# baumgach/PHiSeg-code

Measured on AMD Instinct MI355X. Metric: training images/sec (ELBO step) phiseg_7_5 128x128 LIDC, higher is better.
Workload: dtype bf16; 1 GPU; phiseg_7_5 LIDC 128x128x1, 2 classes, bf16, batch norm, batch 64 per GPU, full ELBO training step (fwd + CE + KL + bwd + Adam); global_batch=64, parallelism=dp1

## Files before the change

include/phx.h:

```cpp
#ifndef PHX_H
#define PHX_H
#include <stddef.h>
#include <stdint.h>

#ifdef __cplusplus
extern "C" {
#endif

enum { PHX_F32 = 0, PHX_BF16 = 1 };
enum { PHX_ACT_ID = 0, PHX_ACT_RELU = 1, PHX_ACT_SOFTPLUS = 2 };
enum { PHX_OK = 0, PHX_E_INVAL = -1, PHX_E_SHAPE = -2, PHX_E_ALIGN = -3, PHX_E_LAUNCH = -4, PHX_E_RUNTIME = -5, PHX_E_COMM = -6 };

int phx_abi_version(void);
int phx_last_error(char* buf, size_t n);
int phx_crc32c(const void* data, size_t n, unsigned* crc);
int phx_device_info(int* cu_count, int* clock_khz, size_t* hbm_bytes, char* name, size_t name_n);
int phx_stream_create(void** stream);
int phx_stream_destroy(void* stream);
int phx_stream_sync(void* stream);
int phx_event_create(void** ev);
int phx_event_destroy(void* ev);
int phx_event_record(void* ev, void* stream);
int phx_event_sync(void* ev);
int phx_event_elapsed_ms(void* start, void* stop, float* ms);
// ... 217 lines not shown
int phx_upconv_supported(int B, int h, int w, int Cin, int Cout);
int phx_upconv_pack(const float* w_hwio, void* weff_fwd, void* weff_dgrad , void* wt_fwd, void* wt_dgrad ,
                    const float* bias, float* bias4, int Cin, int Cout, void* stream);
int phx_upconv_fold_wgrad(const float* dweff, const float* dwt , float* dw_hwio, int Cin, int Cout, void* stream);
int phx_upconv_frame_gather(const void* x, void* f_rows, void* f_cols, int B, int h, int w, int C, void* stream);
int phx_upconv_frame_scatter(const void* fr, const void* fc, void* y_packed, int B, int h, int w, int Cout, void* stream);
int phx_upconv_frame_gather_dy(void* dy_packed, void* dfr, void* dfc, int B, int h, int w, int Cout, void* stream);
int phx_upconv_frame_scatter_dx(const void* df_rows, const void* df_cols, void* dx, int B, int h, int w, int C, void* stream);
int phx_norm_apply_fused_d2s(const void* x, int x_dt, const float* sums, const float* pivot, const float* gamma, const float* beta, float eps,
                             void* y, int y_dt, float* mean, float* rstd, float* scale, float* shift, float* moving_mean, float* moving_var,
                             float momentum, int NS, int P, int C, int G, int act, int h, int w, void* stream);
int phx_norm_bwd_reduce_s2d(const void* dA, int da_dt, const void* x, int x_dt, const float* scale, const float* shift,
                            const float* mean, const float* rstd, float* sums2, int NS, int P, int C, int G, int act, int nrep, int h,
                            int w, void* stream);
int phx_norm_bwd_apply_fused_s2d(const void* dA, int da_dt, const void* x, int x_dt, const float* scale, const float* shift,
                                 const float* mean, const float* rstd, const float* gamma, const float* sums2, void* dx, int dx_dt,
                                 float* dgamma, float* dbeta, const float* fwd_sums, const float* fwd_pivot, float* dbias, int NS, int P,
                                 int C, int G, int act, int nrep, int h, int w, void* stream);
int phx_depth_to_space2(const void* packed, void* hi, int B, int h, int w, int C, void* stream);
int phx_space_to_depth2(const void* hi, void* packed, int B, int h, int w, int C, void* stream);
int phx_bilinear_up2x_fwd(const void* x, int dt, void* y, int B, int h, int w, int C, void* stream);
int phx_bilinear_up2x_bwd(const void* dy, int dt, void* dx, int B, int h, int w, int C, void* stream);
int phx_bilinear_up2x_bwd_acc(const void* dy, int dt, void* dx, int B, int h, int w, int C, void* stream);
int phx_concat2(const void* a, int Ca, const void* b, int Cb, void* out, size_t npix, int dt, void* stream);
int phx_split2(const void* in, void* a, int Ca, void* b, int Cb, size_t npix, int dt, void* stream);
int phx_add_inplace(void* dst, const void* src, size_t n, int dt, void* stream);
int phx_channel_sum_accumulate(const void* x, int dt, float* out, size_t npix, int C, void* stream);
int phx_cast(const void* src, int src_dt, void* dst, int dst_dt, size_t n, void* stream);
int phx_posterior_input(const float* x, const uint8_t* s, void* out, int out_dt, size_t npix, int nlabels,
                        void* stream);
int phx_global_avgpool_fwd(const float* x, float* y, int B, int P, int C, void* stream);
int phx_global_avgpool_bwd(const float* dy, float* dx, int B, int P, int C, void* stream);
int phx_broadcast_pixels_fwd(const float* z, void* out, int out_dt, int B, int P, int C, void* stream);
int phx_broadcast_pixels_bwd(const void* dout, int dt, float* dz, int B, int P, int C, void* stream);
int phx_recomb_samples(const void* feat, int feat_dt, const float* z, const float* W0, const float* W1, const float* W2,
                       const float* W3, const float* b3, const float* s0, const float* t0, const float* s1, const float* t1,
                       const float* s2, const float* t2, float* logits, float* sm, int B, int n, int P, int KF, int K, int Z, int C,
                       void* stream);

int phx_reparam_fwd(const float* mu, const float* sigma, float* z, int B, int per_sample, uint64_t seed,
                    const int32_t* step_dev, int stream_id, int sample_offset, void* stream);
int phx_reparam_bwd(const float* dz, float* dsigma, int B, int per_sample, uint64_t seed,
                    const int32_t* step_dev, int stream_id, int sample_offset, void* stream);
int phx_philox_normal(float* out, int B, int per_sample, uint64_t seed, const int32_t* step_dev, int stream_id,
                      int sample_offset, void* stream);

// ... 112 lines not shown
```

phiseg_code_amd/engine.py:

```python
import ctypes
import os

import numpy as np
import torch

from phiseg_code_amd import graph as G
from phiseg_code_amd import optimizers
from phiseg_code_amd import runtime as rt
from phiseg_code_amd.tfwrapper import normalisation as tfnorm

from phiseg_code_amd.engine_common import *
from phiseg_code_amd.engine_common import (_BN_SMALL, _BN_SMALL_F32, _DETERMINISTIC, _NREP, _NREP_MINP, _fgn_mode, _dual_enabled, _noop,
                                           _device, _TORCH_DT, _NP_DT, _ESIZE, _LIK_SIDE_MAXLVL, _WGRAD_DEFER_BLOCKS, _STAMPS)
from phiseg_code_amd.engine_backward import BackwardLowering
from phiseg_code_amd.engine_forward import ForwardLowering


class ParamStore:

    def __init__(self, graph, seed=0, live=None, optimizer=None):
        self.graph = graph
        self.offset, self.state_offset = {}, {}
        off = soff = 0
        names = list(graph.variables)
# ... 439 lines not shown
        if with_bw:
            self._emit(self.L.memset, self.store.grads.data_ptr(), 0, self.store.grads.numel() * 4, self.stream)
        if self._stamp_tagged:
            for k in range(16):
                self._cur.append((self.L.stamp, (self._tstamp_buf.data_ptr() + 8 * k, self.stream)))
        nl = len(self._lanes)
        self.op_lane = {op: self._lane_of(op) for op in ops}
        opset = set(ops)
        self._opset = opset
        self._lat = self._find_latent_heads(ops)
        self._kl_group = None
        kls = [op for op in ops if op.type == "kl"]
        if len(kls) >= 2 and len(kls) <= 8:
            ws = [self.loss_weight.get(op.outputs[0], 0.0) for op in kls]
            i0, i1 = ops.index(kls[0]), ops.index(kls[-1])
            between = [op for op in ops[i0:i1 + 1] if op.type != "kl"]
            if (len({self.op_lane[op] for op in kls}) == 1 and all(abs(w - ws[0]) < 1e-12 for w in ws)
                    and not any(i.op in kls for b in between for i in b.inputs)):
                self._kl_group = dict(ops=kls, recs=[], gscale=ws[0])
        self._bw_skip = set()
        self._norm_head = {}
        self._pool_done = set()
        self._recomb = self._find_recomb_chains(ops)
        fork = self._record(0) if nl > 1 else None
        for ln in range(1, nl):
            self._lane = ln
            self._wait(fork)
        if nl > 1:
            self._touch = torch.zeros(64, dtype=torch.int64, device=_device())
            self._keep.append(self._touch)
            toks = []
            for ln in range(1, nl):
                self._lane = ln
                self._emit(self.L.stamp, self._touch.data_ptr() + 8 * ln, self.stream)
                toks.append(self._record(ln))
            self._lane = 0
            for evl in toks:
                self._wait(evl)
        self.fw_event = {}
        for op in ops:
            ln = self._lane = self.op_lane[op]
            for t in op.inputs:
                self._wait(self.fw_event.get(self._real_producer(t)))
            n0 = len(self._cur)
            self._stamp_begin()
            if op in self._recomb:
# ... 203 lines not shown
```

phiseg_code_amd/engine_backward.py:

```python
import ctypes

import numpy as np

from phiseg_code_amd import runtime as rt
from phiseg_code_amd import upconv
from phiseg_code_amd.engine_common import *
from phiseg_code_amd.engine_common import _HEAD_RIDER_NOUT, _BN_SMALL, _BN_SMALL_F32, _BN_WIDE, _BN_WIDE_MAXLINES, _DETERMINISTIC, _NREP, _NREP_MINP, _fgn_mode, _dual_enabled, _noop, _device, _TORCH_DT, _NP_DT, _ESIZE, _LIK_SIDE_MAXLVL, _WGRAD_DEFER_BLOCKS, _STAMPS


class BackwardLowering:
    def _bw_l2_weights(self, op):
        st = self.store
        self._emit(self.L.axpy_masked, st.grads.data_ptr(), st.params.data_ptr(), st.decay_mask.data_ptr(), st.n_train,
                   float(self._l2_weight), self.stream)

    def _bw_latent_group(self, rec):
        mu_op, sig_op, add_op = rec["mu"], rec["sig"], rec["add"]
        mu_t, sig_t = mu_op.outputs[0], sig_op.outputs[0]
        for t in (mu_t, sig_t):
            if t in self.grad:
                self._finalize_grad(t)
        dz = self.grad.get(add_op.outputs[0]) if add_op is not None else None
        dmu, dsg = self.grad.get(mu_t), self.grad.get(sig_t)
        for o in (mu_op, sig_op, add_op):
            if o is not None:
                self._bw_skip.add(o)
        if dz is None and dmu is None and dsg is None:
            return
        x_t = rec["x"]
        x, sigma = self.val[x_t], self.val[sig_t]
        npix, cin, zd = rec["npix"], rec["cin"], rec["zd"]
        gmu, gsig = self._alloc((npix, zd), F32), self._alloc((npix, zd), F32)
        st, Lb = self.store, self.L
        wmu, wsg = mu_op.attrs["W"], sig_op.attrs["W"]
        if not self.req.get(x_t, False):
            raise NotImplementedError("latent heads on a tensor without gradient")

        def wr(g):
            self._emit(Lb.latent_heads_bwd, dz.ptr if dz is not None else None, dmu.ptr if dmu is not None else None,
                       dsg.ptr if dsg is not None else None, sigma.ptr, st.ptr(wmu), st.ptr(wsg), g.ptr, g.dt, gmu.ptr, gsig.ptr, npix,
                       cin, zd, rec["hw"], self.rng_seed, self._noise_step_ptr(), rec["sid"], self.sample_offset, self.stream)
        self._add_grad(x_t, write_fn=wr)
        for hop, gy in ((mu_op, gmu), (sig_op, gsig)):
            W, b = hop.attrs["W"], hop.attrs["b"]
# ... 47 lines not shown
            op = op.inputs[0].op
        return op

    def _real_consumers(self, t, opset):
        out = []
        for c in t.consumers:
            if c not in opset:
                continue
            if c.type in self._VIRTUAL:
                for o in c.outputs:
                    out.extend(self._real_consumers(o, opset))
            else:
                out.append(c)
        return out

    def _finalize_grad(self, t):
        for buf, evl in self.pending.pop(t, []):
            self._wait(evl)
            g = self.grad[t]
            if buf is not g:
                assert g.dt == buf.dt and g.n == buf.n
                self._emit(self.L.add_inplace, g.ptr, buf.ptr, g.n, g.dt, self.stream)

    def _bw_placeholder(self, op):
        pass


    _bw_one_hot = _bw_sub_const = _bw_random_normal = _bw_mul = _bw_weighted_sum = _bw_constant = _bw_dice_table = _bw_placeholder

    def _resize_adjoint(self, dfine, dst, add):
        B, h, w, C = dst.shape
        assert dfine.dt == F32 and dst.dt == F32 and dfine.shape[1] % h == 0
        self._emit(self.L.nn_resize_adjoint, dfine.ptr, dst.ptr, B, h, w, C, (dfine.shape[1] // h).bit_length() - 1, int(add), self.stream)

    def _bw_nn_resize(self, op):
        d, src = self.grad[op.outputs[0]], self.val[op.inputs[0]]
        if op.attrs["shift"] == 0:
            return self._add_grad(op.inputs[0], buf=d)
        assert d.shape[1] == src.shape[1] << op.attrs["shift"], "the gradient of a resized tensor is taken at full resolution"
        self._add_grad(op.inputs[0], write_fn=lambda g: self._resize_adjoint(d, g, False), accum_fn=lambda g: self._resize_adjoint(d, g, True))

    def _bw_residual_ce(self, op):
        sv = self.saved.get(op)
        if sv:
            g = self.grad.get(op.outputs[op.attrs["L"]])
            if g is not None:
# ... 23 lines not shown
        sv = self.saved.get(op)
        if sv:
            lg, lab = self.val[op.inputs[0]], self.val[op.inputs[1]]
            B, H, W, C = lg.shape

            def emit(g, add):
                self._emit(self.L.dice_grad, lg.ptr, lab.ptr, sv["coef"].ptr, sv["gscale"], add, g.ptr, B, H, W, C, self.stream)
            self._add_grad(op.inputs[0], write_fn=lambda g: emit(g, 0), accum_fn=lambda g: emit(g, 1))

    def _bw_seg_xent(self, op):
        sv = self.saved.get(op)
        if sv:
            self._add_grad(op.inputs[0], buf=sv["d"])

    def _bw_kl(self, op):
        sv = self.saved.get(op)
        if sv:
            for t, g in zip(op.inputs, sv["gs"]):
                self._add_grad(t, buf=g)

    def _bw_add(self, op):
        if op in self._lat:
            return self._bw_latent_group(self._lat[op])
        sv, dz = self.saved[op], self.grad[op.outputs[0]]
        self._add_grad(sv["mu_t"], buf=dz)
        B = dz.shape[0]

        def wr(target):
            self._emit(self.L.reparam_bwd, dz.ptr, target.ptr, B, sv["per"], self.rng_seed,
                       self._noise_step_ptr(), sv["stream_id"], self.sample_offset, self.stream)
        self._add_grad(sv["sigma_t"], write_fn=wr)

    def _bw_concat(self, op):
        a, b = op.inputs
        d = self.grad[op.outputs[0]]
        if b.op.type == "sub_const":
            return
        npix = int(np.prod(d.shape[:-1]))
        ca, cb = self.val[a].shape[-1], self.val[b].shape[-1]
        da = self._alloc(self.val[a].shape, d.dt) if self.req.get(a) else None
        db = self._alloc(self.val[b].shape, d.dt) if self.req.get(b) else None
        self._emit(self.L.split2, d.ptr, da.ptr if da else None, ca, db.ptr if db else None, cb, npix, d.dt,
                   self.stream)
        for t, g in ((a, da), (b, db)):
            if g is not None:
                self._add_grad(t, buf=self._as_dt(g, self.val[t].dt))
# ... 350 lines not shown
            wsb = int(Lb.conv3x3_mfma_ws_bytes(B, H, Wd, cout, cin))
            ws = self._alloc((wsb // 4,), F32) if wsb else None
            self._emit(Lb.conv3x3_mfma_bf16_ws, dY.ptr, wd.ptr, g.ptr if g is not None else None, None, 0, None, ws.ptr if ws else None, wsb,
                       B, H, Wd, cout, cin, S, **dtag)
            return ws
        if isinstance(x, DualBuf):
            ta, tb = xin.op.inputs
            _, wd = self._packed(W)
            g1, g2 = self._alloc(x.a.shape, BF16), self._alloc(x.b.shape, BF16)
            wsb = int(Lb.conv3x3_mfma_ws_bytes(B, H, Wd, cout, cin))
            ws = self._alloc((wsb // 4,), F32) if wsb else None
            self._emit(Lb.conv3x3_mfma_bf16_dual, dY.ptr, None, 0, wd.ptr, g1.ptr, g2.ptr, x.k1, None, None, 0, None, 0,
                       ws.ptr if ws else None, wsb, B, H, Wd, cout, cin, S, **dtag)
            for t, gb in ((ta, g1), (tb, g2)):
                if self.req.get(t, False):
                    self._add_grad(t, buf=gb)
        elif sv.norm_head:
            self._add_grad(xin, buf=HeadGrad(self.val[xin], dY, self.store.ptr(W), cout))
        elif sv.head1x1:
            self._add_grad(xin, write_fn=lambda g: self._emit(
                Lb.head1x1_dgrad, dY.ptr, self.store.ptr(W), g.ptr, g.dt, B * H * Wd, cin, cout, S))
        elif sv.padded:
            ce, wdp = sv.cin_eff, sv.wd_pad

            def wr(g):
                inplace = ce == cin and g.dt == BF16
                gp = g if inplace else self._alloc((B, H, Wd, ce), BF16)
                self._emit(Lb.conv3x3_mfma_bf16, dY.ptr, wdp.ptr, gp.ptr, None, 0, None, B, H, Wd, cout, ce, S, **dtag)
                if not inplace:
                    self._emit(Lb.unpad_channels_bf16, gp.ptr, g.ptr, g.dt, cin, ce, B * H * Wd, S)
            self._add_grad(xin, write_fn=wr)
        elif sv.mfma and self._slice_grad_ok(op, xin, B, H, Wd, cout, cin):
            _, wd = self._packed(W)
            ws = mfma_dgrad(None)
            self._add_grad(xin, buf=SliceGrad(self.val[xin], ws, int(Lb.conv3x3_mfma_ksplit(B, H, Wd, cout, cin))))
        elif sv.mfma:
            _, wd = self._packed(W)
            self._add_grad(xin, write_fn=mfma_dgrad)
        elif sv.f32m and cin % 32 == 0 and dY.dt == F32 and self._wpk32.get(W.name, (None, None))[1] is not None:
            wd32 = self._wpk32[W.name][1]

            def wr_f32m(g):
                assert g.dt == F32
                self._emit(Lb.conv3x3_f32_mfma, dY.ptr, wd32.ptr, None, g.ptr, B, H, Wd, cout, cin, 0, S,
                           tag="conv3x3_f32_mfma_dgrad", flops=18.0 * cin * cout * B * H * Wd)
            self._add_grad(xin, write_fn=wr_f32m)
# ... 5 lines not shown
```

phiseg_code_amd/engine_common.py:

```python
import ctypes
import enum
import os

import numpy as np
import torch

from phiseg_code_amd import graph as G
from phiseg_code_amd import runtime as rt
from phiseg_code_amd.tfwrapper import normalisation as tfnorm

__all__ = ['F32', 'BF16', 'U8', '_TORCH_DT', '_NP_DT', '_ESIZE', '_LIK_SIDE_MAXLVL', '_WGRAD_DEFER_BLOCKS', '_NREP', '_NREP_MINP', '_STAMPS', '_DETERMINISTIC', '_BN_SMALL', '_BN_SMALL_F32', '_BN_WIDE', '_BN_WIDE_MAXLINES', '_SKIP_HEAD_A', '_POOL_FUSE', '_xf_enabled', '_upconv_min_h', 'UpBuf', '_fgn_mode', '_dual_enabled', '_f32_mfma_enabled', '_recomb_enabled', '_onepass_enabled', '_head_rider_enabled', '_HEAD_RIDER_NOUT', '_noop', '_device', 'live_variables', 'device_sync', 'Buf', 'DualBuf', 'HeadGrad', 'SliceGrad', 'XfBuf', 'NormRoute', 'StatsSource', 'ConvSaved', 'RenormSaved']

F32, BF16, U8 = rt.F32, rt.BF16, 2
_TORCH_DT = {F32: torch.float32, BF16: torch.bfloat16, U8: torch.uint8}
_NP_DT = {F32: np.float32, U8: np.uint8}
_ESIZE = {F32: 4, BF16: 2, U8: 1}
_LIK_SIDE_MAXLVL = 3
_WGRAD_DEFER_BLOCKS = 96
_NREP = 4
_NREP_MINP = 4096
_STAMPS = os.environ.get("PHX_STAMPS", "0") == "1"
_DETERMINISTIC = os.environ.get("PHX_DETERMINISTIC", "0") not in ("0", "")
_BN_SMALL = 1024
_BN_SMALL_F32 = True
_BN_WIDE_MAXLINES = 2048
_SKIP_HEAD_A = True
_POOL_FUSE = True
_BN_WIDE = 2


def _fgn_mode():
    return int(os.environ.get("PHX_FGN", "1"))


def _upconv_min_h():
    return int(os.environ.get("PHX_UPCONV", "64"))


def _xf_enabled():
    return os.environ.get("PHX_XF", "1") == "1"


def _dual_enabled():
    return os.environ.get("PHX_DUAL", "1") == "1"


def _recomb_enabled():
    return os.environ.get("PHX_RECOMB", "1") == "1"


def _f32_mfma_enabled():
    return os.environ.get("PHX_F32_MFMA", "1") == "1"


def _onepass_enabled():
    return os.environ.get("PHX_ONEPASS", "1") == "1"


_HEAD_RIDER_NOUT = (2, 4)


def _head_rider_enabled():
    return os.environ.get("PHX_HEAD_RIDER", "1") != "0"


def _noop():
    pass
# ... 77 lines not shown
    def __init__(self, like, ws, nz):
        self.shape, self.dt, self.n = like.shape, like.dt, like.n
        self.ws, self.nz = ws, nz


class XfBuf:

    def __init__(self, like, y, scale, shift):
        self.shape, self.dt, self.n = like.shape, like.dt, like.n
        self.y, self.scale, self.shift = y, scale, shift


class UpBuf:

    def __init__(self, src, shape):
        self.src, self.shape, self.dt = src, tuple(int(v) for v in shape), src.dt
        self.n = int(np.prod(self.shape))

    @property
    def nbytes(self):
        return self.n * _ESIZE[self.dt]


class RenormSaved:
    __slots__ = ("r", "d", "gamma_eff", "dgs", "dbs")

    def __init__(self, r, d, gamma_eff, dgs=None, dbs=None):
        self.r, self.d, self.gamma_eff, self.dgs, self.dbs = r, d, gamma_eff, dgs, dbs


class NormRoute(enum.Enum):
    NONE, INFER_FOLDED, INFER, BN_WIDE, BN_SMALL_F32Y, BN_SMALL, FGN, NORM_SMALL, GENERIC, RENORM_SMALL = range(10)


class StatsSource(enum.Enum):
    PARTIALS, PARTIALS_NS, ATOMIC, DIRECT, PIVOT_PASS = range(5)


class ConvSaved:
    _OPTIONAL = dict(route=NormRoute.NONE, y=None, scale=None, shift=None, mean=None, rstd=None, NS=None, P=None, G=None, wd_pad=None,
                     upconv=None, a_unwritten=None, fsums=None, fpivot=None, transposed=None, general=None, geo=None, f32m=False,
                     norm_head=False, latent=False, renorm=None)
    __slots__ = ("x", "out", "norm", "mfma", "padded", "cin_eff", "k1", "head1x1") + tuple(_OPTIONAL)

    def __init__(self, x, out, norm, mfma, padded, cin_eff, k1, head1x1, **optional):
        self.x, self.out, self.norm, self.mfma, self.padded, self.cin_eff, self.k1, self.head1x1 = x, out, norm, mfma, padded, cin_eff, k1, head1x1
# ... 9 lines not shown
```

phiseg_code_amd/engine_forward.py:

```python
import ctypes
import types

import numpy as np
import torch

from phiseg_code_amd import graph as G
from phiseg_code_amd import runtime as rt
from phiseg_code_amd import upconv
from phiseg_code_amd.tfwrapper import normalisation as tfnorm
from phiseg_code_amd.engine_common import *
from phiseg_code_amd.engine_common import _BN_SMALL, _BN_SMALL_F32, _BN_WIDE, _BN_WIDE_MAXLINES, _SKIP_HEAD_A, _DETERMINISTIC, _NREP, _NREP_MINP, _fgn_mode, _dual_enabled, _recomb_enabled, _noop, _device, _TORCH_DT, _NP_DT, _ESIZE, _LIK_SIDE_MAXLVL, _WGRAD_DEFER_BLOCKS, _STAMPS


def conv_norm_route(Lb, norm, training, bw, act_dt, x_dt, y_dt, out_dt, B, H, Wd, cin_eff, cout, Gn, mfma, head1x1, concat_free, upsampled,
                    deterministic=_DETERMINISTIC, fgn=None):
    fgn = _fgn_mode() if fgn is None else fgn
    if norm is None:
        return NormRoute.NONE, None
    per_batch = norm in ("batch", "renorm")
    NS, P = (1, B * H * Wd) if per_batch else (B, H * Wd)
    if norm == "batch" and not training:
        return (NormRoute.INFER_FOLDED if (mfma and not head1x1 and not bw) else NormRoute.INFER), None
    both_bf16 = y_dt == BF16 and out_dt == BF16
    if norm == "renorm" and both_bf16 and P <= _BN_SMALL and Lb.renorm_small_supported(P, cout, y_dt, out_dt):
# ... 257 lines not shown
                     for t in (mu.outputs[0], sig.outputs[0]) for c in t.consumers if c in opset)
            ok = ok and len({self.op_lane[o] for o in members}) == 1
            if not ok:
                continue
            rec = dict(mu=mu, sig=sig, add=add, last=last, x=x)
            for o in members:
                out[o] = rec
        return out

    def _fw_latent_group(self, rec):
        mu_op, sig_op, add_op = rec["mu"], rec["sig"], rec["add"]
        x = self.val[rec["x"]]
        mu, sigma = self.val[mu_op.outputs[0]], self.val[sig_op.outputs[0]]
        z = self.val[add_op.outputs[0]] if add_op is not None else None
        cin, zd = mu_op.attrs["W"].shape[-2], mu_op.attrs["W"].shape[-1]
        npix = int(np.prod(x.shape[:-1]))
        hw = npix // x.shape[0]
        sid = add_op.inputs[1].op.inputs[1].op.attrs["stream"] if add_op is not None else 0
        st = self.store
        self._emit(self.L.latent_heads_fwd, x.ptr, x.dt, st.ptr(mu_op.attrs["W"]), st.ptr(mu_op.attrs["b"]), st.ptr(sig_op.attrs["W"]),
                   st.ptr(sig_op.attrs["b"]), mu.ptr, sigma.ptr, z.ptr if z is not None else None, npix, cin, zd, hw, self.rng_seed,
                   self._noise_step_ptr(), sid, self.sample_offset, self.stream)
        rec.update(npix=npix, hw=hw, sid=sid, cin=cin, zd=zd)

    def _find_recomb_chains(self, ops):
        out = {}
        if self.loss is not None or not _recomb_enabled():
            return out
        opset = set(ops)

        def sole_reader(t):
            cons = [c for c in t.consumers if c in opset]
            return cons[0] if (len(cons) == 1 and t not in self.fetches and t not in self.fed) else None

        def plain_1x1(op):
            a = op.attrs
            return (op.type == "conv_unit" and a.get("transposed") is None and a.get("general") is None and a["ksize"] == 1
                    and op not in self._lat)
        for tb in ops:
            if tb.type != "tile_batch" or len(tb.inputs[0].shape) != 4:
                continue
            KF = tb.inputs[0].shape[-1]
            if KF not in (32, 64):
                continue
            cat = sole_reader(tb.outputs[0])
            if cat is None or cat.type != "concat" or cat.inputs[0] is not tb.outputs[0] or cat.inputs[1].op.type != "tile_pixels":
# ... 141 lines not shown
            sv.y = o.y

    def _conv_operands(self, op, bw):
        a = op.attrs
        x = self.val[op.inputs[0]]
        W, b = a["W"], a["b"]
        k, (_, _, cin, cout) = a["ksize"], W.shape
        B, H, Wd = x.shape[0], x.shape[1], x.shape[2]
        out = self._alloc_like(op.outputs[0])
        self.val[op.outputs[0]] = out
        mfma = (self.act_dt == BF16 and x.dt == BF16 and out.dt == BF16 and k == 3 and cin % 32 == 0
                and cout % 32 == 0)
        dual = x if isinstance(x, DualBuf) else None
        assert dual is None or mfma, "concat-free input reached a convolution off the MFMA path"
        up = x if isinstance(x, UpBuf) else None
        xf = x if isinstance(x, XfBuf) else None
        assert xf is None or (mfma and a["norm"] == "batch" and b is None), "unmaterialised activation reached a convolution that cannot re-form it"
        cin_eff = cin
        k1 = k == 1 and cout % 32 == 0
        padded = (self.act_dt == BF16 and out.dt == BF16 and cout % 32 == 0 and
                  ((k == 3 and (cin % 32 != 0 or x.dt != BF16)) or k1))
        if padded:
            cin_eff = (cin + 31) // 32 * 32
            if cin_eff != cin or x.dt != BF16:
                xp = self._alloc((B, H, Wd, cin_eff), BF16)
                self._emit(self.L.pad_channels_bf16, x.ptr, x.dt, cin, xp.ptr, cin_eff, B * H * Wd, self.stream)
                x = xp
            mfma = True
        head1x1 = (k == 1 and out.dt == F32 and cout in (2, 4, 6, 8) and a["norm"] is None and b is not None)
        f32m = bool(not mfma and self.act_dt == F32 and x.dt == F32 and out.dt == F32 and k == 3 and cout % 32 == 0 and _f32_mfma_enabled()
                    and isinstance(x, Buf) and self.L.conv3x3_f32_mfma_supported(B, H, Wd, cin, cout))
        training = a["training"] if isinstance(a["training"], bool) else self.training
        sv = ConvSaved(x, out, self._lowered_norm(a, training), mfma, padded, cin_eff, bool(padded and k1), head1x1, f32m=f32m)
        wptr, wf = self.store.ptr(W), None
        if padded:
            wf = self._alloc((9 * cin_eff * cout,), BF16)
            sv.wd_pad = self._alloc((9 * cin_eff * cout,), BF16) if (bw and self.req.get(op.inputs[0], False)) else None
            self._pack_jobs.append((wptr, wf.ptr, sv.wd_pad.ptr if sv.wd_pad else 0, cin, cin_eff, cout, 1 if k1 else 0))
        elif mfma:
            wf, _ = self._packed(W)
        return types.SimpleNamespace(op=op, a=a, bw=bw, sv=sv, x=x, out=out, W=W, k=k, cin=cin, cout=cout, B=B, H=H, Wd=Wd, dual=dual, up=up, xf=xf,
                                     wf=wf, wptr=wptr, bptr=self.store.ptr(b) if b is not None else None, act=rt.ACT_CODES[a["act"]],
                                     training=training,
                                     y=None, sums=None, pivot=None, stats=None, apply_args=None)

    def _mfma_conv(self, o, y, bias_p, oscale_p, act_code, stats, stats_mode, ws, wsb):
        Lb, x, xf, dual = self.L, o.x, o.xf, o.dual
# ... 276 lines not shown
        mh = _upconv_min_h()
        if not (mh > 0 and bw and self.loss is not None and self.act_dt == BF16 and isinstance(x, Buf) and x.dt == BF16 and len(x.shape) == 4):
            return None
        ot = op.outputs[0]
        cons = self._real_consumers(ot, self._opset)
        if len(cons) != 1 or ot in self.fetches or x.shape[1] < max(mh, 32) or x.shape[2] < max(mh, 32):
            return None
        c = cons[0]
        a = c.attrs if c.type == "conv_unit" else None
        if (a is None or c.inputs[0] is not ot or a["ksize"] != 3 or a.get("transposed") is not None or a.get("general") is not None
                or a["norm"] not in ("batch", "group", "instance") or (a["norm"] == "batch") != (a["b"] is None)
                or self.op_lane.get(c) != self.op_lane.get(op) or c in self._lat):
            return None
        training = a["training"] if isinstance(a["training"], bool) else self.training
        cin, cout = a["W"].shape[-2], a["W"].shape[-1]
        if not training or cin != x.shape[3] or not self.L.upconv_supported(x.shape[0], x.shape[1], x.shape[2], cin, cout):
            return None
        if cin < 4 * cout:
            return None
        return c

    def _fw_bilinear_up(self, op, bw):
        x = self.val[op.inputs[0]]
        if self._upconv_consumer(op, x, bw) is not None:
            self.val[op.outputs[0]] = UpBuf(x, self._cshape(op.outputs[0]))
            return
        out = self._alloc(self._cshape(op.outputs[0]), x.dt)
        self.val[op.outputs[0]] = out
        self._emit(self.L.bilinear_up2x_fwd, x.ptr, x.dt, out.ptr, x.shape[0], x.shape[1], x.shape[2], x.shape[3],
                   self.stream)

    def _fw_add(self, op, bw):
        if op.outputs[0] in self.fed:
            t = op.outputs[0]
            z = self._alloc(self._cshape(t), F32, zero=True)
            self.val[t] = z
            self.feeds[t] = z
            return
        mu_t, m = op.inputs
        if m.op.type != "mul" or m.op.inputs[1].op.type != "random_normal":
            raise NotImplementedError("only z = mu + sigma * random_normal(...) is on the hot path")
        rec = self._lat.get(op)
        if rec is not None:
            self.val[op.outputs[0]] = self._alloc(self.val[mu_t].shape, F32)
            self.saved[op] = dict(latent=True)
            if rec["last"] is op:
                self._fw_latent_group(rec)
            return
        sigma_t, eps_t = m.op.inputs
        mu, sigma = self.val[mu_t], self.val[sigma_t]
        z = self._alloc(mu.shape, F32)
        self.val[op.outputs[0]] = z
        per = mu.n // mu.shape[0]
        stream_id = eps_t.op.attrs["stream"]
        self._emit(self.L.reparam_fwd, mu.ptr, sigma.ptr, z.ptr, mu.shape[0], per, self.rng_seed,
                   self._noise_step_ptr(), stream_id, self.sample_offset, self.stream)
        self.saved[op] = dict(mu_t=mu_t, sigma_t=sigma_t, per=per, stream_id=stream_id)

    def _fw_tile_batch(self, op, bw):
        x = self.val[op.inputs[0]]
        out = self._alloc(self._cshape(op.outputs[0]), x.dt)
        self.val[op.outputs[0]] = out
        n = op.attrs["tile"]
        assert out.shape[0] == x.shape[0] * n
        per = x.n // x.shape[0]
        if (per * _ESIZE[x.dt]) % 16 and x.dt == F32:
            self._emit(self.L.broadcast_pixels_fwd, x.ptr, out.ptr, F32, x.shape[0], n, per, self.stream)
            return
        self._emit(self.L.repeat_batch, x.ptr, out.ptr, x.shape[0], (x.n // x.shape[0]) * _ESIZE[x.dt], n, self.stream)

    def _fw_global_avgpool(self, op, bw):
        x = self._as_dt(self.val[op.inputs[0]], F32)
        out = self._alloc_like(op.outputs[0])
        self.val[op.outputs[0]] = out
        self._emit(self.L.global_avgpool_fwd, x.ptr, out.ptr, x.shape[0], x.shape[1] * x.shape[2], x.shape[3],
                   self.stream)

    def _fw_tile_pixels(self, op, bw):
        z = self.val[op.inputs[0]]
        out = self._alloc_like(op.outputs[0])
# ... 152 lines not shown
```

Before: 6625 images/s.

## Fuse latent z fan-out (pad + bilinear upsample) and gradient fan-in into glue kernels

Adds zglue kernels. In the forward pass, one kernel writes each sampled latent z both as a channel-padded bf16 map and as a 2x bilinear-upsampled padded map, replacing the separate pad_channels and bilinear_up launches that fed the 3x3 convolutions. In the backward pass, the data-gradient outputs of those convolutions are gathered into a single fan-in kernel that applies the upsample adjoint and sums all sources into dz, with cross-lane events. This cuts launches and intermediate buffers on the small latent paths, at the cost of extra engine bookkeeping and cross-lane waits.

```diff
diff --git a/include/phx.h b/include/phx.h
--- a/include/phx.h
+++ b/include/phx.h
@@ -263,6 +263,11 @@
 int phx_bilinear_up2x_fwd(const void* x, int dt, void* y, int B, int h, int w, int C, void* stream);
 int phx_bilinear_up2x_bwd(const void* dy, int dt, void* dx, int B, int h, int w, int C, void* stream);
 int phx_bilinear_up2x_bwd_acc(const void* dy, int dt, void* dx, int B, int h, int w, int C, void* stream);
+enum { PHX_Z_FANIN_MAX = 4 };
+enum { PHX_Z_SRC_DENSE = 0, PHX_Z_SRC_PAD = 1, PHX_Z_SRC_UP = 2 };
+int phx_z_fanout(const float* z, void* zpad, void* zup, int B, int h, int w, int Z, int Cpad, void* stream);
+int phx_z_fanin(const void* const* srcs, const int* kinds, const int* separate, int nsrc, float* dz, int B, int h, int w, int Z, int Cpad,
+                void* stream);
 int phx_concat2(const void* a, int Ca, const void* b, int Cb, void* out, size_t npix, int dt, void* stream);
 int phx_split2(const void* in, void* a, int Ca, void* b, int Cb, size_t npix, int dt, void* stream);
 int phx_add_inplace(void* dst, const void* src, size_t n, int dt, void* stream);
diff --git a/phiseg_code_amd/csrc/zglue.hip b/phiseg_code_amd/csrc/zglue.hip
--- /dev/null
+++ b/phiseg_code_amd/csrc/zglue.hip
@@ -0,0 +1,281 @@
+#include "phx_common.h"
+
+template <int Z>
+__device__ __forceinline__ void zg_load_f32(const float* __restrict__ p, float o[Z]) {
+    const float2* q = reinterpret_cast<const float2*>(p);
+#pragma unroll
+    for (int j = 0; j < Z / 2; ++j) {
+        const float2 t = q[j];
+        o[2 * j] = t.x;
+        o[2 * j + 1] = t.y;
+    }
+}
+template <int Z>
+__device__ __forceinline__ void zg_load_pad(const unsigned short* __restrict__ p, float o[Z]) {
+    const uint4 r = *reinterpret_cast<const uint4*>(p);
+    const unsigned w[4] = {r.x, r.y, r.z, r.w};
+#pragma unroll
+    for (int j = 0; j < Z / 2; ++j) {
+        o[2 * j] = __uint_as_float(w[j] << 16);
+        o[2 * j + 1] = __uint_as_float(w[j] & 0xffff0000u);
+    }
+}
+template <int Z>
+__device__ __forceinline__ uint4 zg_chunk0(const float v[Z]) {
+    unsigned w[4] = {0u, 0u, 0u, 0u};
+#pragma unroll
+    for (int j = 0; j < Z / 2; ++j) w[j] = (unsigned)f2bf(v[2 * j]) | ((unsigned)f2bf(v[2 * j + 1]) << 16);
+    return make_uint4(w[0], w[1], w[2], w[3]);
+}
+
+template <int Z>
+__global__ void k_z_fanout(const float* __restrict__ z, unsigned short* __restrict__ zpad, unsigned short* __restrict__ zup, int B, int h,
+                           int w, int Cpad) {
+    const int Q = Cpad / 8, OW = 2 * w;
+    const size_t items = (size_t)B * h * w * Q;
+    for (size_t it = blockIdx.x * (size_t)blockDim.x + threadIdx.x; it < items; it += (size_t)gridDim.x * blockDim.x) {
+        const int q = (int)(it % Q);
+        size_t r = it / Q;
+        const size_t pix = r;
+        const int x0 = (int)(r % w); r /= w;
+        const int y0 = (int)(r % h);
+        const size_t base = (r / h) * h;
+        uint4 c00 = make_uint4(0u, 0u, 0u, 0u), c01 = c00, c10 = c00, c11 = c00, cz = c00;
+        if (q == 0) {
+            float a[Z];
+            zg_load_f32<Z>(z + pix * Z, a);
+            cz = zg_chunk0<Z>(a);
+            if (zup) {
+                const int y1 = min(y0 + 1, h - 1), x1 = min(x0 + 1, w - 1);
+                float bb[Z], c[Z], d[Z], o00[Z], o01[Z], o10[Z], o11[Z];
+                zg_load_f32<Z>(z + ((base + y0) * w + x1) * Z, bb);
+                zg_load_f32<Z>(z + ((base + y1) * w + x0) * Z, c);
+                zg_load_f32<Z>(z + ((base + y1) * w + x1) * Z, d);
+#pragma unroll
+                for (int j = 0; j < Z; ++j) {
+                    const float top = fmaf(bb[j] - a[j], 0.5f, a[j]);
+                    const float bot = fmaf(d[j] - c[j], 0.5f, c[j]);
+                    o00[j] = fmaf(c[j] - a[j], 0.f, a[j]);
+                    o01[j] = fmaf(bot - top, 0.f, top);
+                    o10[j] = fmaf(c[j] - a[j], 0.5f, a[j]);
+                    o11[j] = fmaf(bot - top, 0.5f, top);
+                }
+                c00 = zg_chunk0<Z>(o00);
+                c01 = zg_chunk0<Z>(o01);
+                c10 = zg_chunk0<Z>(o10);
+                c11 = zg_chunk0<Z>(o11);
+            }
+        }
+        if (zpad) *reinterpret_cast<uint4*>(zpad + pix * Cpad + (size_t)q * 8) = cz;
+        if (zup) {
+            const size_t o = ((base * 2 + 2 * y0) * OW + 2 * x0) * Cpad + (size_t)q * 8;
+            *reinterpret_cast<uint4*>(zup + o) = c00;
+            *reinterpret_cast<uint4*>(zup + o + Cpad) = c01;
+            *reinterpret_cast<uint4*>(zup + o + (size_t)OW * Cpad) = c10;
+            *reinterpret_cast<uint4*>(zup + o + (size_t)OW * Cpad + Cpad) = c11;
+        }
+    }
+}
+
+struct ZFanInArgs {
+    const void* src[PHX_Z_FANIN_MAX];
+    int kind[PHX_Z_FANIN_MAX];
+    int separate[PHX_Z_FANIN_MAX];
+    int n;
+};
+
+template <int Z>
+__device__ __forceinline__ void zg_adjoint(const unsigned short* __restrict__ dy, int b, int iy, int ix, int h, int w, int Cpad, float acc[Z]) {
+    const int OH = 2 * h, OW = 2 * w;
+    int ty[3], tx[3];
+    float wy[3], wx[3];
+    ty[0] = 2 * iy; wy[0] = 1.f;
+    ty[1] = 2 * iy + 1; wy[1] = (iy == h - 1) ? 1.f : 0.5f;
+    ty[2] = 2 * iy - 1; wy[2] = (iy >= 1) ? 0.5f : 0.f;
+    tx[0] = 2 * ix; wx[0] = 1.f;
+    tx[1] = 2 * ix + 1; wx[1] = (ix == w - 1) ? 1.f : 0.5f;
+    tx[2] = 2 * ix - 1; wx[2] = (ix >= 1) ? 0.5f : 0.f;
+    for (int a = 0; a < 3; ++a) {
+        if (wy[a] == 0.f) continue;
+        for (int c = 0; c < 3; ++c) {
+            if (wx[c] == 0.f) continue;
+            float v[Z];
+            zg_load_pad<Z>(dy + (((size_t)b * OH + ty[a]) * OW + tx[c]) * Cpad, v);
+            const float ww = wy[a] * wx[c];
+#pragma unroll
+            for (int j = 0; j < Z; ++j) acc[j] = fmaf(ww, v[j], acc[j]);
+        }
+    }
+}
+
+template <int Z>
+__global__ void k_z_fanin(const ZFanInArgs A, float* __restrict__ dz, int B, int h, int w, int Cpad) {
+    const size_t items = (size_t)B * h * w;
+    for (size_t it = blockIdx.x * (size_t)blockDim.x + threadIdx.x; it < items; it += (size_t)gridDim.x * blockDim.x) {
+        size_t r = it;
+        const int ix = (int)(r % w); r /= w;
+        const int iy = (int)(r % h);
+        const int b = (int)(r / h);
+        float acc[Z];
+#pragma unroll
+        for (int j = 0; j < Z; ++j) acc[j] = 0.f;
+        for (int k = 0; k < A.n; ++k) {
+            if (A.kind[k] == PHX_Z_SRC_UP) {
+                const unsigned short* dy = (const unsigned short*)A.src[k];
+                if (k == 0 || !A.separate[k]) {
+                    zg_adjoint<Z>(dy, b, iy, ix, h, w, Cpad, acc);
+                } else {
+                    float t[Z];
+#pragma unroll
+                    for (int j = 0; j < Z; ++j) t[j] = 0.f;
+                    zg_adjoint<Z>(dy, b, iy, ix, h, w, Cpad, t);
+#pragma unroll
+                    for (int j = 0; j < Z; ++j) acc[j] = acc[j] + t[j];
+                }
+            } else {
+                float v[Z];
+                if (A.kind[k] == PHX_Z_SRC_DENSE) zg_load_f32<Z>((const float*)A.src[k] + it * Z, v);
+                else zg_load_pad<Z>((const unsigned short*)A.src[k] + it * Cpad, v);
+#pragma unroll
+                for (int j = 0; j < Z; ++j) acc[j] = k == 0 ? v[j] : acc[j] + v[j];
+            }
+        }
+        float2* o = reinterpret_cast<float2*>(dz + it * Z);
+#pragma unroll
+        for (int j = 0; j < Z / 2; ++j) o[j] = make_float2(acc[2 * j], acc[2 * j + 1]);
+    }
+}
+
+template <int Z, int NS>
+__global__ void __launch_bounds__(64) k_z_fanin_pk(const ZFanInArgs A, float* __restrict__ dz, int B, int h, int w, int Cpad) {
+    const size_t items = (size_t)B * h * w;
+    for (size_t it = blockIdx.x * (size_t)blockDim.x + threadIdx.x; it < items; it += (size_t)gridDim.x * blockDim.x) {
+        size_t r = it;
+        const int ix = (int)(r % w); r /= w;
+        const int iy = (int)(r % h);
+        const int b = (int)(r / h);
+        const int ty[3] = {2 * iy, 2 * iy + 1, max(2 * iy - 1, 0)}, tx[3] = {2 * ix, 2 * ix + 1, max(2 * ix - 1, 0)};
+        const float wy[3] = {1.f, (iy == h - 1) ? 1.f : 0.5f, (iy >= 1) ? 0.5f : 0.f};
+        const float wx[3] = {1.f, (ix == w - 1) ? 1.f : 0.5f, (ix >= 1) ? 0.5f : 0.f};
+        uint4 raw[NS][9];
+#pragma unroll
+        for (int k = 0; k < NS; ++k) {
+            const bool up = A.kind[k] == PHX_Z_SRC_UP;
+            const unsigned short* p = (const unsigned short*)A.src[k];
+            const int HH = up ? 2 * h : h, WW = up ? 2 * w : w;
+#pragma unroll
+            for (int a = 0; a < 3; ++a)
+#pragma unroll
+                for (int c = 0; c < 3; ++c) {
+                    const int yy = up ? ty[a] : iy, xx = up ? tx[c] : ix;
+                    raw[k][3 * a + c] = *reinterpret_cast<const uint4*>(p + (((size_t)b * HH + yy) * WW + xx) * Cpad);
+                }
+        }
+        float acc[Z];
+#pragma unroll
+        for (int j = 0; j < Z; ++j) acc[j] = 0.f;
+#pragma unroll
+        for (int k = 0; k < NS; ++k) {
+            const bool up = A.kind[k] == PHX_Z_SRC_UP, own = up && k > 0 && A.separate[k];
+            float t[Z];
+#pragma unroll
+            for (int j = 0; j < Z; ++j) t[j] = (up && !own) ? acc[j] : 0.f;
+            if (up) {
+#pragma unroll
+                for (int a = 0; a < 3; ++a)
+#pragma unroll
+                    for (int c = 0; c < 3; ++c) {
+                        const float ww = wy[a] * wx[c];
+                        const unsigned wd[4] = {raw[k][3 * a + c].x, raw[k][3 * a + c].y, raw[k][3 * a + c].z, raw[k][3 * a + c].w};
+                        if (wy[a] != 0.f && wx[c] != 0.f) {
+#pragma unroll
+                            for (int j = 0; j < Z / 2; ++j) {
+                                t[2 * j] = fmaf(ww, __uint_as_float(wd[j] << 16), t[2 * j]);
+                                t[2 * j + 1] = fmaf(ww, __uint_as_float(wd[j] & 0xffff0000u), t[2 * j + 1]);
+                            }
+                        }
+                    }
+            } else {
+                const unsigned wd[4] = {raw[k][0].x, raw[k][0].y, raw[k][0].z, raw[k][0].w};
+#pragma unroll
+                for (int j = 0; j < Z / 2; ++j) {
+                    t[2 * j] = __uint_as_float(wd[j] << 16);
+                    t[2 * j + 1] = __uint_as_float(wd[j] & 0xffff0000u);
+                }
+            }
+#pragma unroll
+            for (int j = 0; j < Z; ++j) acc[j] = (k == 0 || (up && !own)) ? t[j] : acc[j] + t[j];
+        }
+        float2* o = reinterpret_cast<float2*>(dz + it * Z);
+#pragma unroll
+        for (int j = 0; j < Z / 2; ++j) o[j] = make_float2(acc[2 * j], acc[2 * j + 1]);
+    }
+}
+
+#define PHX_Z_SWITCH(Z, ZC, ...)                  \
+    do {                                           \
+        if ((Z) == 2) { constexpr int ZC = 2; __VA_ARGS__; }      \
+        else if ((Z) == 4) { constexpr int ZC = 4; __VA_ARGS__; } \
+        else { constexpr int ZC = 6; __VA_ARGS__; }               \
+    } while (0)
+
+static int zglue_domain(int B, int h, int w, int Z, int Cpad) {
+    PHX_REQUIRE(B >= 1 && h >= 1 && w >= 1, PHX_E_INVAL, "z glue: empty map");
+    PHX_REQUIRE(Z == 2 || Z == 4 || Z == 6, PHX_E_INVAL, "z glue: Z must be 2, 4 or 6");
+    PHX_REQUIRE(Cpad == 32, PHX_E_INVAL, "z glue: Cpad must be 32");
+    return PHX_OK;
+}
+
+extern "C" {
+
+int phx_z_fanout(const float* z, void* zpad, void* zup, int B, int h, int w, int Z, int Cpad, void* stream) {
+    const int rc = zglue_domain(B, h, w, Z, Cpad);
+    if (rc != PHX_OK) return rc;
+    PHX_REQUIRE(z != NULL && (zpad != NULL || zup != NULL), PHX_E_INVAL, "z_fanout: z and at least one output");
+    PHX_REQUIRE(((uintptr_t)z & 7) == 0 && (((uintptr_t)zpad | (uintptr_t)zup) & 15) == 0, PHX_E_ALIGN, "z_fanout: z 8-byte, outputs 16-byte aligned");
+    const size_t items = (size_t)B * h * w * (Cpad / 8);
+    PHX_Z_SWITCH(Z, ZC, {
+        hipLaunchKernelGGL((k_z_fanout<ZC>), dim3(phx_grid_for(items, 256)), dim3(256), 0, (hipStream_t)stream, z, (unsigned short*)zpad,
+                           (unsigned short*)zup, B, h, w, Cpad);
+    });
+    PHX_CHECK_LAUNCH();
+    return PHX_OK;
+}
+
+int phx_z_fanin(const void* const* srcs, const int* kinds, const int* separate, int nsrc, float* dz, int B, int h, int w, int Z, int Cpad,
+                void* stream) {
+    const int rc = zglue_domain(B, h, w, Z, Cpad);
+    if (rc != PHX_OK) return rc;
+    PHX_REQUIRE(srcs != NULL && kinds != NULL && separate != NULL && dz != NULL && nsrc >= 1 && nsrc <= PHX_Z_FANIN_MAX, PHX_E_INVAL,
+                "z_fanin: 1 to PHX_Z_FANIN_MAX sources");
+    PHX_REQUIRE(((uintptr_t)dz & 7) == 0, PHX_E_ALIGN, "z_fanin: dz 8-byte aligned");
+    ZFanInArgs A;
+    memset(&A, 0, sizeof(A));
+    A.n = nsrc;
+    for (int k = 0; k < nsrc; ++k) {
+        PHX_REQUIRE(srcs[k] != NULL && kinds[k] >= PHX_Z_SRC_DENSE && kinds[k] <= PHX_Z_SRC_UP, PHX_E_INVAL, "z_fanin: bad source");
+        PHX_REQUIRE(((uintptr_t)srcs[k] & (kinds[k] == PHX_Z_SRC_DENSE ? 7 : 15)) == 0, PHX_E_ALIGN,
+                    "z_fanin: dense sources 8-byte, padded sources 16-byte aligned");
+        A.src[k] = srcs[k];
+        A.kind[k] = kinds[k];
+        A.separate[k] = separate[k] != 0;
+    }
+    const size_t items = (size_t)B * h * w;
+    bool dense = false;
+    for (int k = 0; k < nsrc; ++k) dense = dense || kinds[k] == PHX_Z_SRC_DENSE;
+    static_assert(PHX_Z_FANIN_MAX == 4, "the dispatch below lists the source counts");
+    const dim3 grid(phx_grid_for(items, 64)), block(64);
+#define PHX_Z_FANIN_PK(NSC) hipLaunchKernelGGL((k_z_fanin_pk<ZC, NSC>), grid, block, 0, (hipStream_t)stream, A, dz, B, h, w, Cpad)
+    PHX_Z_SWITCH(Z, ZC, {
+        if (dense) hipLaunchKernelGGL((k_z_fanin<ZC>), grid, block, 0, (hipStream_t)stream, A, dz, B, h, w, Cpad);
+        else if (nsrc == 1) PHX_Z_FANIN_PK(1);
+        else if (nsrc == 2) PHX_Z_FANIN_PK(2);
+        else if (nsrc == 3) PHX_Z_FANIN_PK(3);
+        else PHX_Z_FANIN_PK(4);
+    });
+#undef PHX_Z_FANIN_PK
+    PHX_CHECK_LAUNCH();
+    return PHX_OK;
+}
+
+}
diff --git a/phiseg_code_amd/engine.py b/phiseg_code_amd/engine.py
--- a/phiseg_code_amd/engine.py
+++ b/phiseg_code_amd/engine.py
@@ -485,6 +485,7 @@
         self._norm_head = {}
         self._pool_done = set()
         self._recomb = self._find_recomb_chains(ops)
+        self._zg, self._zg_conv, self._zg_up = self._find_zglue(ops)
         fork = self._record(0) if nl > 1 else None
         for ln in range(1, nl):
             self._lane = ln
diff --git a/phiseg_code_amd/engine_backward.py b/phiseg_code_amd/engine_backward.py
--- a/phiseg_code_amd/engine_backward.py
+++ b/phiseg_code_amd/engine_backward.py
@@ -20,6 +20,8 @@
         for t in (mu_t, sig_t):
             if t in self.grad:
                 self._finalize_grad(t)
+        if add_op is not None:
+            self._zglue_fanin(add_op.outputs[0])
         dz = self.grad.get(add_op.outputs[0]) if add_op is not None else None
         dmu, dsg = self.grad.get(mu_t), self.grad.get(sig_t)
         for o in (mu_op, sig_op, add_op):
@@ -113,6 +115,29 @@
                 assert g.dt == buf.dt and g.n == buf.n
                 self._emit(self.L.add_inplace, g.ptr, buf.ptr, g.n, g.dt, self.stream)
 
+    def _zglue_source(self, rec, gp, how):
+        t, srcs, lane = rec["t"], rec["sources"], self._lane
+        primary = not srcs or (how == "up" and all(s["lane"] == lane for s in srcs if s["primary"]))
+        evl = self._record(lane) if len(self._lanes) > 1 else None
+        srcs.append(dict(buf=gp, kind=2 if how == "up" else 1, primary=primary, lane=lane, evl=evl))
+        if t not in self.grad:
+            self.grad[t] = self._alloc(self.val[t].shape, F32)
+
+    def _zglue_fanin(self, t):
+        rec = self._zg.get(t)
+        if rec is None or not rec["sources"]:
+            return
+        srcs = [s for s in rec["sources"] if s["primary"]] + [s for s in rec["sources"] if not s["primary"]]
+        rec["sources"] = []
+        for s in srcs:
+            self._wait(s["evl"])
+        dz = self.grad[t]
+        B, h, w, Z = dz.shape
+        ptrs, kinds = rt.ptr_array([s["buf"].ptr for s in srcs]), rt.int_array([s["kind"] for s in srcs])
+        sep = rt.int_array([0 if s["primary"] else 1 for s in srcs])
+        self._keep += [ptrs, kinds, sep]
+        self._emit(self.L.z_fanin, ptrs, kinds, sep, len(srcs), dz.ptr, B, h, w, Z, 32, self.stream)
+
     def _bw_placeholder(self, op):
         pass
 
@@ -182,6 +207,7 @@
     def _bw_add(self, op):
         if op in self._lat:
             return self._bw_latent_group(self._lat[op])
+        self._zglue_fanin(op.outputs[0])
         sv, dz = self.saved[op], self.grad[op.outputs[0]]
         self._add_grad(sv["mu_t"], buf=dz)
         B = dz.shape[0]
@@ -578,6 +604,11 @@
                 Lb.head1x1_dgrad, dY.ptr, self.store.ptr(W), g.ptr, g.dt, B * H * Wd, cin, cout, S))
         elif sv.padded:
             ce, wdp = sv.cin_eff, sv.wd_pad
+            zg = self._zg_conv.get(op)
+            if zg is not None and zg[0]["bw"]:
+                gp = self._alloc((B, H, Wd, ce), BF16)
+                self._emit(Lb.conv3x3_mfma_bf16, dY.ptr, wdp.ptr, gp.ptr, None, 0, None, B, H, Wd, cout, ce, S, **dtag)
+                return self._zglue_source(zg[0], gp, zg[1])
 
             def wr(g):
                 inplace = ce == cin and g.dt == BF16
diff --git a/phiseg_code_amd/engine_common.py b/phiseg_code_amd/engine_common.py
--- a/phiseg_code_amd/engine_common.py
+++ b/phiseg_code_amd/engine_common.py
@@ -9,7 +9,7 @@
 from phiseg_code_amd import runtime as rt
 from phiseg_code_amd.tfwrapper import normalisation as tfnorm
 
-__all__ = ['F32', 'BF16', 'U8', '_TORCH_DT', '_NP_DT', '_ESIZE', '_LIK_SIDE_MAXLVL', '_WGRAD_DEFER_BLOCKS', '_NREP', '_NREP_MINP', '_STAMPS', '_DETERMINISTIC', '_BN_SMALL', '_BN_SMALL_F32', '_BN_WIDE', '_BN_WIDE_MAXLINES', '_SKIP_HEAD_A', '_POOL_FUSE', '_xf_enabled', '_upconv_min_h', 'UpBuf', '_fgn_mode', '_dual_enabled', '_f32_mfma_enabled', '_recomb_enabled', '_onepass_enabled', '_head_rider_enabled', '_HEAD_RIDER_NOUT', '_noop', '_device', 'live_variables', 'device_sync', 'Buf', 'DualBuf', 'HeadGrad', 'SliceGrad', 'XfBuf', 'NormRoute', 'StatsSource', 'ConvSaved', 'RenormSaved']
+__all__ = ['F32', 'BF16', 'U8', '_TORCH_DT', '_NP_DT', '_ESIZE', '_LIK_SIDE_MAXLVL', '_WGRAD_DEFER_BLOCKS', '_NREP', '_NREP_MINP', '_STAMPS', '_DETERMINISTIC', '_BN_SMALL', '_BN_SMALL_F32', '_BN_WIDE', '_BN_WIDE_MAXLINES', '_SKIP_HEAD_A', '_POOL_FUSE', '_xf_enabled', '_upconv_min_h', 'UpBuf', '_fgn_mode', '_dual_enabled', '_f32_mfma_enabled', '_recomb_enabled', '_zglue_enabled', 'ZUpBuf', '_onepass_enabled', '_head_rider_enabled', '_HEAD_RIDER_NOUT', '_noop', '_device', 'live_variables', 'device_sync', 'Buf', 'DualBuf', 'HeadGrad', 'SliceGrad', 'XfBuf', 'NormRoute', 'StatsSource', 'ConvSaved', 'RenormSaved']
 
 F32, BF16, U8 = rt.F32, rt.BF16, 2
 _TORCH_DT = {F32: torch.float32, BF16: torch.bfloat16, U8: torch.uint8}
@@ -43,6 +43,10 @@
 
 def _dual_enabled():
     return os.environ.get("PHX_DUAL", "1") == "1"
+
+
+def _zglue_enabled():
+    return os.environ.get("PHX_ZGLUE", "1") == "1"
 
 
 def _recomb_enabled():
@@ -166,6 +170,13 @@
         return self.n * _ESIZE[self.dt]
 
 
+class ZUpBuf:
+
+    def __init__(self, pad, shape):
+        self.pad, self.shape, self.dt = pad, tuple(int(v) for v in shape), F32
+        self.n = int(np.prod(self.shape))
+
+
 class RenormSaved:
     __slots__ = ("r", "d", "gamma_eff", "dgs", "dbs")
 
diff --git a/phiseg_code_amd/engine_forward.py b/phiseg_code_amd/engine_forward.py
--- a/phiseg_code_amd/engine_forward.py
+++ b/phiseg_code_amd/engine_forward.py
@@ -303,6 +303,61 @@
                    st.ptr(sig_op.attrs["b"]), mu.ptr, sigma.ptr, z.ptr if z is not None else None, npix, cin, zd, hw, self.rng_seed,
                    self._noise_step_ptr(), sid, self.sample_offset, self.stream)
         rec.update(npix=npix, hw=hw, sid=sid, cin=cin, zd=zd)
+        if add_op is not None:
+            self._zglue_fanout(add_op.outputs[0])
+
+    def _find_zglue(self, ops):
+        zg, by_conv, by_up = {}, {}, {}
+        if not _zglue_enabled() or self.act_dt != BF16:
+            return zg, by_conv, by_up
+        opset = self._opset
+
+        def reader_ok(c, t, Z):
+            a = c.attrs
+            return (c.type == "conv_unit" and c not in self._lat and a.get("transposed") is None and a.get("general") is None
+                    and a["ksize"] == 3 and c.inputs[0] is t and a["W"].shape[-2] == Z and a["W"].shape[-1] % 32 == 0
+                    and self._dt_of(c.outputs[0]) == BF16)
+        for op in ops:
+            t = op.outputs[0] if op.type == "add" else None
+            if t is None or t.kind != G.KIND_F32 or len(t.shape) != 4 or t.shape[-1] not in (2, 4, 6):
+                continue
+            Z, pad, up, other = t.shape[-1], [], [], 0
+            for c in t.consumers:
+                if c not in opset:
+                    continue
+                if reader_ok(c, t, Z):
+                    pad.append(c)
+                    continue
+                if c.type == "bilinear_up" and c.inputs[0] is t and c.outputs[0] not in self.fetches:
+                    cons = self._real_consumers(c.outputs[0], opset)
+                    if len(cons) == 1 and reader_ok(cons[0], c.outputs[0], Z) and self.op_lane.get(cons[0]) == self.op_lane.get(c):
+                        up.append((c, cons[0]))
+                        continue
+                other += 1
+            if not pad and not up:
+                continue
+            rec = zg[t] = dict(t=t, Z=Z, zpad=None, zup=None, want_pad=bool(pad), want_up=bool(up), sources=[],
+                               bw=bool(self.loss is not None and other == 0 and len(pad) + len(up) <= 4))
+            for c in pad:
+                by_conv[c] = (rec, "pad")
+            for u, c in up:
+                by_conv[c] = (rec, "up")
+                by_up[u] = rec
+        return zg, by_conv, by_up
+
+    def _zglue_fanout(self, t):
+        rec = self._zg.get(t)
+        if rec is None:
+            return
+        z = self.val[t]
+        B, h, w, Z = z.shape
+        assert z.dt == F32
+        if rec["want_pad"]:
+            rec["zpad"] = self._alloc((B, h, w, 32), BF16)
+        if rec["want_up"]:
+            rec["zup"] = self._alloc((B, 2 * h, 2 * w, 32), BF16)
+        self._emit(self.L.z_fanout, z.ptr, rec["zpad"].ptr if rec["zpad"] is not None else None,
+                   rec["zup"].ptr if rec["zup"] is not None else None, B, h, w, Z, 32, self.stream)
 
     def _find_recomb_chains(self, ops):
         out = {}
@@ -490,7 +545,11 @@
                   ((k == 3 and (cin % 32 != 0 or x.dt != BF16)) or k1))
         if padded:
             cin_eff = (cin + 31) // 32 * 32
-            if cin_eff != cin or x.dt != BF16:
+            zg = self._zg_conv.get(op)
+            if zg is not None:
+                x = zg[0]["zup" if zg[1] == "up" else "zpad"]
+                assert x is not None and x.shape == (B, H, Wd, cin_eff)
+            elif cin_eff != cin or x.dt != BF16:
                 xp = self._alloc((B, H, Wd, cin_eff), BF16)
                 self._emit(self.L.pad_channels_bf16, x.ptr, x.dt, cin, xp.ptr, cin_eff, B * H * Wd, self.stream)
                 x = xp
@@ -813,6 +872,10 @@
 
     def _fw_bilinear_up(self, op, bw):
         x = self.val[op.inputs[0]]
+        zrec = self._zg_up.get(op)
+        if zrec is not None:
+            self.val[op.outputs[0]] = ZUpBuf(zrec["zup"], self._cshape(op.outputs[0]))
+            return
         if self._upconv_consumer(op, x, bw) is not None:
             self.val[op.outputs[0]] = UpBuf(x, self._cshape(op.outputs[0]))
             return
@@ -827,6 +890,7 @@
             z = self._alloc(self._cshape(t), F32, zero=True)
             self.val[t] = z
             self.feeds[t] = z
+            self._zglue_fanout(t)
             return
         mu_t, m = op.inputs
         if m.op.type != "mul" or m.op.inputs[1].op.type != "random_normal":
@@ -847,6 +911,7 @@
         self._emit(self.L.reparam_fwd, mu.ptr, sigma.ptr, z.ptr, mu.shape[0], per, self.rng_seed,
                    self._noise_step_ptr(), stream_id, self.sample_offset, self.stream)
         self.saved[op] = dict(mu_t=mu_t, sigma_t=sigma_t, per=per, stream_id=stream_id)
+        self._zglue_fanout(op.outputs[0])
 
     def _fw_tile_batch(self, op, bw):
         x = self.val[op.inputs[0]]
```

Result: no change. 6656 images/s, median of 6 (+0.5%).
